# wsakobe/CylinderTag

Measured on AMD Instinct MI355X. Metric: frames/sec detect() 1920x1080, higher is better.
Workload: dtype u8; 1 GPU; synthetic 1920x1080 random-stripe frames, 4096 per step over 1 GPU(s), 4 planted CTag_2f12c markers each, detect(img,5,true,5), inputs resident in HBM; frames_per_gpu=4096, chunk=4096, parallelism=frames sharded, dp1, gather=none (1 GPU)

## Files before the change

### __graft_entry__.py

```python
import os
import subprocess
import sys

ROOT = os.path.dirname(os.path.abspath(__file__))
if ROOT not in sys.path:
    sys.path.insert(0, ROOT)


def build():
    subprocess.check_call(["make", "-s", "-j4", "-C", os.path.join(ROOT, "cylindertag_amd")])
    for name, extra in (("hedge", "-DCTAG_WELSCH_MINERR_IN_LOOP -DCTAG_RESIZE_SIMD_LANES=16"), ("plainsync", "-DCTAG_REFINE_PLAIN_SYNC=1")):
        out = os.path.join("_var", name)
        subprocess.check_call(["make", "-s", "-j4", "-C", os.path.join(ROOT, "cylindertag_amd"), "OUT=" + out, "EXTRA=" + extra, os.path.join(out, "libctag_hip.so")])
    subprocess.check_call(["make", "-s", "-C", os.path.join(ROOT, "testkit")])
    subprocess.check_call(["make", "-s", "-C", os.path.join(ROOT, "oracle")])
    if os.path.isdir("/root/reference"):
        subprocess.call(["make", "-s", "-C", os.path.join(ROOT, "oracle"), "ref"])
    import cylindertag_amd
    from cylindertag_amd import capi
    L = capi.load_library()
    missing = [s for s in capi.EXPORTS if not hasattr(L, s)]
    if missing:
        raise RuntimeError("libctag_hip.so lacks symbols: %s" % missing)
    import testkit
    T = testkit.load_library()
    missing = [s for s in testkit.EXPORTS if not hasattr(T, s)]
# ... 48 lines not shown
```

### cylindertag_amd/csrc/ctag_internal.h

```cpp
#pragma once
#include <hip/hip_runtime.h>
#include <stddef.h>
#include <stdint.h>

#include <vector>

#include "../../include/ctag_types.h"

struct ctag_handle;
struct ctag_camera;
struct ctag_pose_rec;
struct ctag_rig_pose_rec;
struct ctag_mv_pose_rec;
struct ctag_camera_set;

namespace ctag {
template <class T>
struct DevBuf {
    T* p = nullptr;
    size_t cap = 0;
    DevBuf() = default;
    DevBuf(const DevBuf&) = delete;
    DevBuf& operator=(const DevBuf&) = delete;
    ~DevBuf() { release(); }
// ... 292 lines not shown
ChunkPlan plan_chunk(const PlanIn& in);

hipError_t launch_zero_counters(const ChunkPlan& pl, const Workspace& ws, hipStream_t s);
hipError_t launch_decimate(const ChunkPlan& pl, const uint8_t* frames, ptrdiff_t frame_stride, ptrdiff_t row_stride, const Workspace& ws, hipStream_t s);
hipError_t launch_threshold_ccl(const ChunkPlan& pl, const Workspace& ws, hipStream_t s);
hipError_t launch_seam_merge(const ChunkPlan& pl, const Workspace& ws, hipStream_t s);
hipError_t launch_resolve(const ChunkPlan& pl, const Workspace& ws, hipStream_t s);
hipError_t launch_candidates(const ChunkPlan& pl, const Workspace& ws, hipStream_t s);
hipError_t launch_quads(const ChunkPlan& pl, const Workspace& ws, hipStream_t s, hipEvent_t* ev5 = nullptr);
hipError_t launch_line_fits(const ChunkPlan& pl, const Workspace& ws, hipStream_t s, unsigned long long* stamps = nullptr, hipEvent_t ev_sorted = nullptr);
int welsch_limits(int32_t* out, int capacity);
hipError_t launch_features(const ChunkPlan& pl, const Workspace& ws, const DetectParams& p, hipStream_t s);
hipError_t launch_edge_refine(const ChunkPlan& pl, const uint8_t* frames, ptrdiff_t frame_stride, ptrdiff_t row_stride, const Workspace& ws, const DetectParams& p, hipStream_t s);
hipError_t launch_edge_refine_sums(const ChunkPlan& pl, const Workspace& ws, hipStream_t s);
hipError_t launch_markers(const ChunkPlan& pl, const Workspace& ws, const DetectParams& p, ctag_frame_result* out, const PendingCtx& pend, hipStream_t s);
hipError_t launch_counters(int nframes, const Workspace& ws, const ctag_frame_result* results, long long* out10, hipStream_t s);
size_t threshold_ccl_lds_bytes(int tw);
bool build_threshold_table(float dark_cap, uint8_t* table , int* dim, int* tcap);
void build_pick_table(uint8_t* table, uint16_t* table16);


enum SiblingState { kPoseState, kDrawState, kRigState, kGatherState, kMvState, kCovState, kFitState, kRigFitState, kCamFitState, kIntrFitState, kRobustState, kTrackState, kHandEyeState, kNumSiblingStates };
void** handle_state_slot(struct ::ctag_handle* h, SiblingState which, void (*free_fn)(void*));
int model_to_device(struct ::ctag_model* m, int device);
int rigs_to_device(struct ::ctag_rigs* r, int device);
bool camera_ok(const struct ::ctag_camera* c);
bool handle_timing(const struct ::ctag_handle* h);
int handle_finish_pending(struct ::ctag_handle* h);
bool handle_pending_state(struct ::ctag_handle* h, const int32_t** count_dev, uint64_t* gen);
void handle_pending_clean(struct ::ctag_handle* h, uint64_t gen);
// ... 46 lines not shown
```

### cylindertag_amd/csrc/k_feature.hip

```cpp
#include "ctag_internal.h"
#include "ctag_math.h"
#include "ctag_refine.h"
#include "ctag_wave.h"

namespace ctag {

constexpr double kPi = 3.1415926535897932384626433832795;

struct P2 {
    float x, y;
};
__device__ __forceinline__ float dist2p(P2 a, P2 b) { return ctm::sqrt32((a.x - b.x) * (a.x - b.x) + (a.y - b.y) * (a.y - b.y)); }
__device__ __forceinline__ double angdeg(float dy, float dx) { return ctm::atan2_32(dy, dx) * 180 / kPi; }

struct QuadDerived {
    float cx, cy, d[4], a1, a2;
    float e[4];
};
static_assert(sizeof(QuadDerived) == 48, "workspace carve in ctag_api.hip");
struct FeatPtrs {
    const int32_t* ncand;
    const QuadOut* quads;
    QuadDerived* derived;
    int32_t* quad_index;
// ... 377 lines not shown
        f2[k] = F;
    }
    clk.mark(5);
}

struct RefinePtrs {
    const uint8_t* frames;
    ptrdiff_t frame_stride, row_stride;
    const int32_t* nfeat;
    const int32_t* status;
    const FeatureDev* feat1;
    FeatureDev* feat2;
    double* n0;
    int32_t* frame_long;
    int ch;
};
static RefinePtrs refine_ptrs(const uint8_t* frames, ptrdiff_t frame_stride, ptrdiff_t row_stride, const Workspace& ws, const DetectParams& p) {
    RefinePtrs P{};
    P.frames = frames, P.frame_stride = frame_stride, P.row_stride = row_stride, P.ch = p.channels == 3 ? 3 : 1;
    P.nfeat = ws.nfeat, P.status = ws.status, P.feat1 = ws.feat1, P.feat2 = ws.feat2, P.n0 = ws.refine_n0, P.frame_long = ws.frame_long;
    return P;
}
constexpr int kRefineSamples = 128;
constexpr int kRefineThreads = 2 * kRefineSamples;
#ifndef CTAG_REFINE_STAGE_DEEP
#define CTAG_REFINE_STAGE_DEEP 12
#endif
#ifndef CTAG_REFINE_REGION
#define CTAG_REFINE_REGION 21504
#endif
constexpr int kRefineRegion = CTAG_REFINE_REGION;
#ifndef CTAG_REFINE_REGION_LARGE
#define CTAG_REFINE_REGION_LARGE 49152
#endif
constexpr int kRefineRegionLarge = CTAG_REFINE_REGION_LARGE;

#ifndef CTAG_REFINE_SEARCH_WAVES
#define CTAG_REFINE_SEARCH_WAVES 4
#endif
__device__ __forceinline__ void refine_line(const double* A, double* L) {
    const double Mx = A[0], My = A[1], Mxx = A[2], Mxy = A[3], Myy = A[4], N = A[5];
    const ctm::Recip64 RN = ctm::recip64(N);
    const double Ex = ctm::div64(Mx, RN), Ey = ctm::div64(My, RN);
    const double Cxx = ctm::div64(Mxx, RN) - Ex * Ex;
    const double Cxy = ctm::div64(Mxy, RN) - Ex * Ey;
    const double Cyy = ctm::div64(Myy, RN) - Ey * Ey;
    const double normal_theta = .5 * ctm::atan2_32((float)(-2 * Cxy), (float)(Cyy - Cxx));
    L[0] = Ex;
    L[1] = Ey;
    float sn, cs;
    ctm::sincos32((float)normal_theta, &sn, &cs);
// ... 15 lines not shown
        O->c[2 * idx] = (float)(Ln[0] + L0 * A00);
        O->c[2 * idx + 1] = (float)(Ln[1] + L0 * A10);
    } else {
        O->c[2 * idx] = F->c[2 * idx];
        O->c[2 * idx + 1] = F->c[2 * idx + 1];
    }
}

#if defined(CTAG_REFINE_PLAIN_SYNC) && CTAG_REFINE_PLAIN_SYNC
__device__ __forceinline__ void refine_sync() { __syncthreads(); }
__device__ __forceinline__ void sums_sync() { __syncthreads(); }
#else
__device__ __forceinline__ void refine_sync() { lds_barrier(); }
__device__ __forceinline__ void sums_sync() { lds_wait(), __builtin_amdgcn_s_waitcnt(0xc07f); }
#endif
template <int MODE, int REGION = kRefineRegion>
__device__ __forceinline__ bool refine_quad(const RefinePtrs& P, int rows, int cols, int subpix, int frame, int qidx, int only_long, double alpha128 = 0.0) {
    constexpr int kPitch = kRefineSamples + 1;
    constexpr int kRows = 16;
#ifndef CTAG_ONES_SHIFT
#define CTAG_ONES_SHIFT 16
#endif
    __shared__ __attribute__((aligned(16))) double s_vall[MODE == 1 ? kPitch : (kRows + 1) * kPitch + CTAG_ONES_SHIFT];
    double (*s_v)[kPitch] = reinterpret_cast<double (*)[kPitch]>(s_vall);
    double* const s_ones = MODE == 1 ? s_vall : s_vall + kRows * kPitch + CTAG_ONES_SHIFT;
    double (*s_bx)[kPitch] = s_v, (*s_by)[kPitch] = s_v + (MODE == 1 ? 0 : 4);
    __shared__ double s_nrm[4][2];
    __shared__ uint64_t s_step[4][2];
    __shared__ double s_acc[48];
    __shared__ __attribute__((aligned(16))) uint8_t s_reg[REGION];
    const int fi = qidx >> 1, quad = qidx & 1;
    const int tid = threadIdx.x;
    const FeatureDev* F = P.feat1 + (size_t)frame * CTAG_MAX_FEATURES + fi;
    const uint8_t* __restrict__ img = P.frames + (ptrdiff_t)frame * P.frame_stride;
    const uint32_t rs = (uint32_t)P.row_stride;
    const int off = quad * 4;
    __shared__ float s_cx[4], s_cy[4];
    __shared__ int s_ns[4];
    __shared__ int s_box[4];
    if (tid < 4) {
        s_cx[tid] = F->c[2 * (off + tid)];
        s_cy[tid] = F->c[2 * (off + tid) + 1];
    }
    double* const accp = s_acc;
    if (MODE != 1 && tid < 48) accp[tid] = 0.0;
    if constexpr (MODE != 1) {
        for (int k = tid; k < kPitch; k += (int)blockDim.x) s_ones[k] = 1.0;
    }
    refine_sync();
    if (tid < 4) {
        const int a = tid, b = (tid + 1) & 3;
        const double nx = s_cy[b] - s_cy[a];
        const double ny = -s_cx[b] + s_cx[a];
        const double mag = ctm::sqrt64(nx * nx + ny * ny);
        const double ns_d = mag / 8 > 128.0 ? mag / 8 : 128.0;
        s_ns[tid] = (int)ns_d;
        s_nrm[tid][0] = nx / mag;
        s_nrm[tid][1] = ny / mag;
        s_step[tid][0] = ctr::fast_step(nx / mag);
        s_step[tid][1] = ctr::fast_step(ny / mag);
    }
    if (tid == 64) {
        const float m = (float)(subpix + 3);
        const float fx0 = fminf(fminf(s_cx[0], s_cx[1]), fminf(s_cx[2], s_cx[3])) - m, fx1 = fmaxf(fmaxf(s_cx[0], s_cx[1]), fmaxf(s_cx[2], s_cx[3])) + m;
        const float fy0 = fminf(fminf(s_cy[0], s_cy[1]), fminf(s_cy[2], s_cy[3])) - m, fy1 = fmaxf(fmaxf(s_cy[0], s_cy[1]), fmaxf(s_cy[2], s_cy[3])) + m;
        int staged = 0, bx0 = 0, by0 = 0, pitch = 4;
        if (fx0 > -1e6f && fx1 < 1e6f && fy0 > -1e6f && fy1 < 1e6f) {
            bx0 = max((int)floorf(fx0), 0) & ~3;
            by0 = max((int)floorf(fy0), 0);
            const int bx1 = min((int)floorf(fx1) + 1, cols - 1), by1 = min((int)floorf(fy1) + 1, rows - 1);
            if (bx1 >= bx0 && by1 >= by0) {
                pitch = (bx1 - bx0 + 4) & ~3;
                if (((pitch >> 2) & 1) == 0) pitch += 4;
                staged = ((long long)pitch * (by1 - by0 + 1) <= REGION && (pitch >> 2) <= kRefineThreads) ? by1 - by0 + 1 : 0;
            }
        }
        s_box[0] = bx0;
        s_box[1] = by0;
        s_box[2] = pitch;
        s_box[3] = staged;
    }
    refine_sync();
    const int max_ns = max(max(s_ns[0], s_ns[1]), max(s_ns[2], s_ns[3]));
    {
        const bool long_quad = max_ns > kRefineSamples;
        if (MODE == 1 && long_quad && tid == 0) P.frame_long[frame] = 1;
        if (MODE != 0 && long_quad) return false;
        if (MODE == 0 && only_long && !long_quad) return false;
    }
    const int box_x0 = s_box[0], box_y0 = s_box[1], box_pitch = s_box[2], box_rows = s_box[3];
    const bool staged = box_rows > 0;
    if (staged) {
        const int wpr = box_pitch >> 2;
        const int rpp = kRefineThreads / wpr;
        const bool aligned = ((rs & 3u) == 0u) && ((reinterpret_cast<uintptr_t>(img) & 3u) == 0u);
        const int r0 = tid / wpr, c4 = (tid - r0 * wpr) * 4;
        const int gx = box_x0 + c4;
        if (rpp > 0 && r0 < rpp) {
            auto stage_rows = [&](auto load, auto conv) {
                int r = r0;
                if constexpr (MODE == 1) {
                    constexpr int kDeep = CTAG_REFINE_STAGE_DEEP;
                    for (; r + (kDeep - 1) * rpp < box_rows; r += kDeep * rpp) {
                        decltype(load(0)) v[kDeep];
#pragma unroll
                        for (int u = 0; u < kDeep; u++) v[u] = load(r + u * rpp);
#pragma unroll
                        for (int u = 0; u < kDeep; u++) *reinterpret_cast<uint32_t*>(s_reg + (r + u * rpp) * box_pitch + c4) = conv(v[u]);
                    }
                }
                for (; r + 3 * rpp < box_rows; r += 4 * rpp) {
                    const auto v0 = load(r), v1 = load(r + rpp), v2 = load(r + 2 * rpp), v3 = load(r + 3 * rpp);
                    *reinterpret_cast<uint32_t*>(s_reg + r * box_pitch + c4) = conv(v0);
                    *reinterpret_cast<uint32_t*>(s_reg + (r + rpp) * box_pitch + c4) = conv(v1);
                    *reinterpret_cast<uint32_t*>(s_reg + (r + 2 * rpp) * box_pitch + c4) = conv(v2);
                    *reinterpret_cast<uint32_t*>(s_reg + (r + 3 * rpp) * box_pitch + c4) = conv(v3);
                }
                for (; r < box_rows; r += rpp) *reinterpret_cast<uint32_t*>(s_reg + r * box_pitch + c4) = conv(load(r));
            };
            auto same = [](uint32_t v) -> uint32_t { return v; };
            if (P.ch == 3) {
                struct W3 {
                    uint32_t a, b, c;
                };
                if (aligned && box_x0 + box_pitch <= cols) {
                    stage_rows(
                        [&](int r) -> W3 {
                            const uint32_t* src = reinterpret_cast<const uint32_t*>(img + (size_t)__umul24((unsigned)(box_y0 + r), rs) + 3 * gx);
                            return W3{src[0], src[1], src[2]};
                        },
                        [](const W3& w) -> uint32_t { return gray4_of(w.a, w.b, w.c); });
                } else {
                    stage_rows(
                        [&](int r) -> uint32_t {
                            const uint8_t* src = img + (size_t)__umul24((unsigned)(box_y0 + r), rs) + 3 * gx;
                            uint32_t v = 0;
// ... 22 lines not shown
    const int half = tid >> 7, st = tid & (kRefineSamples - 1);
    double* const n0_quad = P.n0 + ((size_t)frame * (CTAG_MAX_FEATURES * 2) + qidx) * (4 * kRefineSamples);
    for (int sbase = 0; sbase < max_ns; sbase += kRefineSamples) {
        const int s = sbase + st;
#pragma nounroll
        for (int epair = 0; epair < 2; epair++) {
            const int edge = 2 * epair + half;
            const int a = edge, b = (edge + 1) & 3;
            const float ax = s_cx[a], ay = s_cy[a], bx = s_cx[b], by = s_cy[b];
            const int nsamples = s_ns[edge];
            const double nx = s_nrm[edge][0], ny = s_nrm[edge][1];
            const bool axis = nx == 0.0 || ny == 0.0;
            const uint64_t step_xy[2] = {s_step[edge][0], s_step[edge][1]};
            bool ok = false;
            double bestx = 0, besty = 0, alpha = 0;
            if (s < nsamples) {
                alpha = MODE == 1 ? alpha128 : (15.0 + s) / (nsamples + 30);
                const double x0 = alpha * ax + (1 - alpha) * bx;
                const double y0 = alpha * ay + (1 - alpha) * by;
                double Mn = 0, Mcount = 0;
                const bool bgr = P.ch == 3;
                auto px = [&](int x, int y) -> unsigned {
                    if (bgr) {
                        const uint8_t* q = img + __umul24((unsigned)y, rs) + 3u * (unsigned)x;
                        return gray_of(q[0], q[1], q[2]);
                    }
                    return img[__umul24((unsigned)y, rs) + (unsigned)x];
                };
                bool done = false;
                if (subpix <= ctr::kFastMaxSubpix && ctr::interior(x0, y0, nx, ny, subpix, rows, cols)) {
                    if (staged) {
                        auto px_lds = [&](int x, int y) -> unsigned { return s_reg[__umul24((unsigned)y, (unsigned)box_pitch) + (unsigned)x]; };
                        if (!axis)
                            done = subpix == 5 ? ctr::search_fast<5>(x0, y0, nx, ny, 5, px_lds, Mn, Mcount, box_x0, box_y0, step_xy)
                                               : ctr::search_fast<0>(x0, y0, nx, ny, subpix, px_lds, Mn, Mcount, box_x0, box_y0, step_xy);
                        if (!done) {
                            ctr::search_mid<0>(x0, y0, nx, ny, subpix, px_lds, Mn, Mcount, box_x0, box_y0);
                            done = true;
                        }
                    } else {
                        done = ctr::search_fast(x0, y0, nx, ny, subpix, px, Mn, Mcount);
                    }
                }
                if (!done) ctr::search_exact(x0, y0, nx, ny, subpix, rows, cols, px, Mn, Mcount);
                if (Mcount != 0) {
                    const double n0 = Mn / Mcount;
                    bestx = x0 + n0 * nx;
                    besty = y0 + n0 * ny;
                    ok = true;
                    if constexpr (MODE == 1) n0_quad[edge * kRefineSamples + st] = n0;
                }
            }
            if constexpr (MODE == 1) {
                if (!ok) n0_quad[edge * kRefineSamples + st] = ctm::bits_to_f64(0x7ff8000000000000ULL);
            } else {
                s_bx[edge][st] = bestx;
                s_by[edge][st] = besty;
                s_v[8 + edge][st] = ok ? 1 - alpha : 0.0;
                s_v[12 + edge][st] = ok ? alpha : 0.0;
            }
        }
        if constexpr (MODE == 1) return false;
        refine_sync();
        if (tid < 48) {
            const int edge = tid / 12, r = tid - edge * 12;
// ... 12 lines not shown
            }
            for (; k < cntS; k++) acc += (pa[k] * pb[k]) * pw[k];
            accp[tid] = acc;
        }
        refine_sync();
    }
    if (tid < 8) {
        const int edge = tid >> 1, pass = tid & 1;
        refine_line(s_acc + edge * 12 + pass * 6, s_acc + edge * 12 + pass * 6);
    }
    refine_sync();
    if (tid < 4) refine_corner(s_acc, tid, off, F, P.feat2 + (size_t)frame * CTAG_MAX_FEATURES + fi);
    return true;
}

template <int MODE, int REGION = kRefineRegion>
__global__ __launch_bounds__(kRefineThreads) __attribute__((amdgpu_waves_per_eu(MODE == 1 ? (REGION > 36864 ? 3 : CTAG_REFINE_SEARCH_WAVES) : 1, MODE == 1 ? CTAG_REFINE_SEARCH_WAVES : 8)))
void k_edge_refine(RefinePtrs P, int rows, int cols, int subpix, int nframes, int per_frame) {
    int frame = blockIdx.y, bx = blockIdx.x, gx = gridDim.x;
    if (per_frame > 0) {
        const int b = blockIdx.x;
        frame = ((b >> 3) / per_frame) * 8 + (b & 7);
        bx = (b >> 3) % per_frame;
        gx = per_frame;
    }
    if (frame >= nframes) return;
    if (P.status[frame] != CTAG_OK) return;
    const int nq = 2 * min(P.nfeat[frame], CTAG_MAX_FEATURES);
    const double alpha128 = (15.0 + (double)((int)threadIdx.x & (kRefineSamples - 1))) / (kRefineSamples + 30);
    for (int q = bx; q < nq; q += gx) {
        refine_quad<MODE, REGION>(P, rows, cols, subpix, frame, q, 0, alpha128);
        if (q + gx < nq) refine_sync();
    }
}
#ifndef CTAG_REFINE_SUMS2_WAVES
#define CTAG_REFINE_SUMS2_WAVES 4
#endif
constexpr int kSumSeg = 16, kSumSegs = kRefineSamples / kSumSeg;
constexpr int kSumPitch = kSumSeg + 2;
constexpr int kSumRows = 24;
struct SumsWeights {
    double w[kRefineSamples][2];
    constexpr SumsWeights() : w{} {
        for (int s = 0; s < kRefineSamples; s++) {
            const double alpha = (15.0 + s) / (kRefineSamples + 30);
            w[s][0] = 1 - alpha;
// ... 838 lines not shown
            }
            out_markers++;
            out_features += rn;
        }
        clk.mark(24);
    }
    if (tid == 0) {
        out->status = CTAG_OK;
        out->n_markers = out_markers;
        out->n_features = out_features;
        out->flags = oflags;
    }
}

static Stamps feat_stamps;

hipError_t launch_features(const ChunkPlan& pl, const Workspace& ws, const DetectParams& p, hipStream_t s) {
    const FeatPtrs P = feat_ptrs(ws, pl.feat_stamps ? feat_stamps.zeroed(s) : nullptr);
    if (pl.latency) hipLaunchKernelGGL(k_features<512>, dim3(pl.nframes), dim3(512), 0, s, P, pl.nframes, p.feature_size);
    else hipLaunchKernelGGL(k_features<128>, dim3(pl.nframes), dim3(128), 0, s, P, pl.nframes, p.feature_size);
    return hipGetLastError();
}
static void launch_refine_sums(const ChunkPlan& pl, const RefinePtrs& P, hipStream_t s) {
    const int f8 = ((pl.nframes + 7) / 8) * 8;
    hipLaunchKernelGGL(k_edge_refine_sums, dim3(f8 * pl.refine_sums_gx), dim3(64), 0, s, P, pl.nframes, pl.refine_sums_gx);
}
hipError_t launch_edge_refine_sums(const ChunkPlan& pl, const Workspace& ws, hipStream_t s) {
    launch_refine_sums(pl, refine_ptrs(nullptr, 0, 0, ws, DetectParams{}), s);
    return hipGetLastError();
}
hipError_t launch_edge_refine(const ChunkPlan& pl, const uint8_t* frames, ptrdiff_t frame_stride, ptrdiff_t row_stride, const Workspace& ws, const DetectParams& p, hipStream_t s) {
    const int nframes = pl.nframes, refine_gx = pl.refine_gx, f8 = ((nframes + 7) / 8) * 8;
    const RefinePtrs P = refine_ptrs(frames, frame_stride, row_stride, ws, p);
    if (pl.refine == RefineForm::None) return hipSuccess;
    if (pl.refine == RefineForm::One) {
        hipLaunchKernelGGL(k_edge_refine<0>, dim3(CTAG_MAX_FEATURES * 2, nframes), dim3(kRefineThreads), 0, s, P, ws.g.rows, ws.g.cols, p.subpix_dist, nframes, 0);
        return hipGetLastError();
    }
    if (pl.refine == RefineForm::SplitLarge) hipLaunchKernelGGL((k_edge_refine<1, kRefineRegionLarge>), dim3(f8 * refine_gx), dim3(kRefineThreads), 0, s, P, ws.g.rows, ws.g.cols, p.subpix_dist, nframes, refine_gx);
    else if (pl.refine == RefineForm::SplitLooping) hipLaunchKernelGGL(k_edge_refine<1>, dim3(f8 * refine_gx), dim3(kRefineThreads), 0, s, P, ws.g.rows, ws.g.cols, p.subpix_dist, nframes, refine_gx);
    else hipLaunchKernelGGL(k_edge_refine<1>, dim3(refine_gx, nframes), dim3(kRefineThreads), 0, s, P, ws.g.rows, ws.g.cols, p.subpix_dist, nframes, 0);
    launch_refine_sums(pl, P, s);
    hipLaunchKernelGGL(k_edge_refine_tail, dim3(13, nframes), dim3(64), 0, s, P, nframes, 13);
    hipLaunchKernelGGL(k_edge_refine_long, dim3(4, nframes), dim3(kRefineThreads), 0, s, P, ws.g.rows, ws.g.cols, p.subpix_dist, nframes);
    return hipGetLastError();
}
hipError_t launch_markers(const ChunkPlan& pl, const Workspace& ws, const DetectParams& p, ctag_frame_result* out, const PendingCtx& pend, hipStream_t s) {
    const MarkerPtrs P = marker_ptrs(ws, p, out, pend, pl.feat_stamps ? feat_stamps.d : nullptr);
    if (pl.latency) hipLaunchKernelGGL(k_markers<8>, dim3(pl.nframes), dim3(512), 0, s, P, pl.nframes, p.feature_size, p.dict_rows, p.dict_cols);
    else hipLaunchKernelGGL(k_markers<1>, dim3(pl.nframes), dim3(64), 0, s, P, pl.nframes, p.feature_size, p.dict_rows, p.dict_cols);
    if (pl.feat_stamps) {
        unsigned long long h[25];
        feat_stamps.read(s, h, 25);
        fprintf(stderr, "[k_features ticks] compact %llu derive %llu pairs %llu greedy %llu organise %llu obtain %llu\n", h[0], h[1], h[2], h[3], h[4], h[5]);
        fprintf(stderr, "[k_markers ticks] load %llu pairs %llu union %llu sort %llu ids %llu carry+pre %llu | code %llu coverage %llu pick+store %llu\n", h[16], h[17], h[18],
                h[19], h[20], h[21], h[22], h[23], h[24]);
    }
    return hipGetLastError();
}

}
```

### include/ctag_testkit.h

```cpp
#ifndef CTAG_TESTKIT_H
#define CTAG_TESTKIT_H
#include <stddef.h>
#include <stdint.h>

#include "ctag.h"
#include "ctag_pose.h"

#ifdef __cplusplus
extern "C" {
#endif

#define CTAG_DBG_HALF 1
#define CTAG_DBG_LABELS 2
#define CTAG_DBG_CANDIDATES 3
#define CTAG_DBG_CAND_QUADS 4
#define CTAG_DBG_FEATURES0 5
#define CTAG_DBG_FEATURES1 6
#define CTAG_DBG_FEATURES2 7
#define CTAG_DBG_PREMARKERS 8
#define CTAG_DBG_GRAY 9
#define CTAG_DBG_MASK 11
#define CTAG_DBG_LINES 10
#define CTAG_DBG_LINE_POINTS 12
#define CTAG_DBG_LINE_FITS 13
// ... 72 lines not shown
                            ctag_synth3d_truth* truth);
int ctag_synth3d_model(const int32_t* state, int dict_rows, int dict_cols, float* corners);

int ctag_testkit_dense_edge_probe(ctag_handle* h, const uint8_t* gray, int rows, int cols, ptrdiff_t row_stride, const double* segments,
                                  int n_seg, const double* K, const double* dist, const double* rvec, const double* tvec,
                                  int samples_per_edge, double search_px, double min_contrast, double* out, int32_t* keep);

int ctag_testkit_welsch_fit(ctag_handle* h, int n_frames, const int32_t* edges_per_frame, const int32_t* points_per_edge, const int32_t* xy,
                            int latency, int welsch_gx, int welsch_gs, int tail_at_pool_end, float* lines);

int ctag_testkit_welsch_limits(int32_t* out, int capacity);

int ctag_testkit_refine_sums(ctag_handle* h, int n_frames, const int32_t* nfeat, const int32_t* status, const float* corners, const double* n0,
                             double* sums);

int ctag_testkit_model_fit_system(ctag_handle* h, const ctag_frame_result* results, int n_frames, const ctag_pose_rec* poses, int n_poses,
                                  const ctag_model* model, const ctag_camera* camera, int model_index, double lambda, int min_obs, int pass_records,
                                  double* S, double* g, double* delta, int32_t* held, int32_t* bad_pivot);
int ctag_testkit_model_fit_limits(int32_t* out, int capacity);

int ctag_testkit_rig_fit_system(ctag_handle* h, const ctag_frame_result* results, int n_frames, const ctag_rig_pose_rec* rig_poses,
                                const ctag_model* model, const ctag_rigs* rigs, const ctag_camera* camera, int rig, double lambda, int pass_records,
                                double* S, double* g, double* delta, int32_t* n_unknowns, int32_t* bad_pivot);
int ctag_testkit_rig_fit_limits(int32_t* out, int capacity);

int ctag_testkit_camera_fit_system(ctag_handle* h, const ctag_frame_result* results, int n_frames, const ctag_mv_pose_rec* mv_poses,
                                   const ctag_model* model, const ctag_rigs* rigs, const ctag_camera_set* cams, int anchor, double lambda,
                                   int pass_records, double* S, double* g, double* delta, int32_t* n_unknowns, int32_t* bad_pivot);
int ctag_testkit_camera_fit_limits(int32_t* out, int capacity);

// ... 16 lines not shown
```

### testkit/__init__.py

```python
import ctypes as C
import os
import subprocess

import numpy as np

import cylindertag_amd as ca
from cylindertag_amd import capi
from cylindertag_amd.capi import CtagError, Model

_HERE = os.path.dirname(os.path.abspath(__file__))
_LIB = os.environ.get("CTAG_TESTKIT_LIB") or os.path.join(_HERE, "_build", "libctag_testkit.so")

TRUTH3D_DT = np.dtype([("n_markers", "<i4"), ("dict_row", "<i4", (8,)), ("_pad", "<i4", (1,)), ("R", "<f8", (8, 9)), ("t", "<f8", (8, 3)),
                       ("radius", "<f8", (8,))])
TRUTH_DT = np.dtype([("n_markers", "<i4"), ("dict_row", "<i4", (8,)), ("strip_len", "<f4", (8,)),
                     ("corners", "<f4", (8, 8))])
DBG_HALF, DBG_LABELS, DBG_CANDIDATES, DBG_CAND_QUADS, DBG_FEATURES0, DBG_FEATURES1, DBG_FEATURES2, DBG_PREMARKERS, DBG_GRAY, DBG_LINES, DBG_MASK, DBG_LINE_POINTS, DBG_LINE_FITS, DBG_PACKS, DBG_PACKS1 = range(1, 16)
SYNTH_SEED = 0x4354616753594E00

EXPORTS = ["ctag_debug_fetch", "ctag_math_probe", "ctag_testkit_wave_probe", "ctag_testkit_exp32_k0_sweep", "ctag_testkit_unpack_gathered", "ctag_testkit_stall_stream", "ctag_synth_frames_device", "ctag_synth_frame_host",
           "ctag_synth_layout_truth", "ctag_synth3d_frames_device", "ctag_synth3d_frame_host", "ctag_synth3d_model",
           "ctag_testkit_dense_edge_probe", "ctag_testkit_plan", "ctag_testkit_welsch_fit", "ctag_testkit_welsch_limits", "ctag_testkit_refine_sums",
           "ctag_testkit_model_fit_system", "ctag_testkit_model_fit_limits", "ctag_testkit_rig_fit_system", "ctag_testkit_rig_fit_limits",
           "ctag_testkit_camera_fit_system", "ctag_testkit_camera_fit_limits",
           "ctag_testkit_intrinsics_fit_system", "ctag_testkit_intrinsics_fit_poses", "ctag_testkit_intrinsics_fit_limits"]
PLAN_FIELDS = ("fused", "bgr_direct", "zero_first", "dec_zero_kernel", "dec_zero_list", "dec", "dec_xblocks", "dec_yblocks", "dec_band_rows", "dec_bands",
               "ccl", "latency", "small_cfg", "refprm", "mask_scan", "prescan", "all_wave", "fork", "pack_max", "big_points", "pack_gx", "scan_gx",
               "mscan_gx", "big_cols", "big_max_gx", "welsch_gs", "welsch_gx", "refine", "refine_gx", "refine_sums_gx")
DEC_FORMS = ("mask", "mask_bands", "general", "wide", "banded135", "banded", "unaligned")
CCL_FORMS = ("mask", "tw5", "any")
WELSCH_LIMITS = ("kWShort", "kWCap", "kWRes", "kWPts", "kWPtsU", "kPickN", "kPickN2", "kWE", "kWT", "kLatLines", "kLatPoints", "kLatChunk", "kLdsLines",
                 "kLatencyFrames", "kLatRankBlocks", "kLineSortBuckets")
REFINE_FORMS = ("none", "one", "split_large", "split_looping", "split")
MATH_EXP32_NONPOS, MATH_EXP32_NONPOS_K0, MATH_LOG64 = 15, 17, 18
WAVE_OPS = ("FROM_PREV", "FROM_NEXT", "SHR1_I32", "SHR2_I32", "SHR4_I32", "SHR1_F32", "SHR1_F64", "XOR1_I32", "XOR2_I32", "HALF_MIRROR_I32", "ROW_MIRROR_I32",
            "XOR1_I64", "XOR2_I64", "HALF_MIRROR_I64", "ROW_MIRROR_I64", "INCL_SCAN", "SG_SUM8_I32", "SG_SUM64_I32", "SG_SUM8_I64", "SG_SUM64_I64",
            "SG_BEST8_NEAREST", "SG_BEST8_FARTHEST", "SG_BEST64_NEAREST", "SG_BEST64_FARTHEST", "SUM_F64", "MAX_F64", "ALL", "PK_MIN_U16", "PK_MAX_U16")
for _i, _n in enumerate(WAVE_OPS):
    globals()["WAVE_" + _n] = _i
WAVE_SENTINEL_F64, WAVE_SENTINEL_I64 = -12345.6789, -0x5a5a5a5a5a5a5a5a


def lib_path():
    return _LIB


def build(verbose=False):
# ... 39 lines not shown
    L.ctag_synth3d_frame_host.restype = C.c_int
    L.ctag_synth3d_frame_host.argtypes = [i32p, C.c_int, C.c_int, vp, C.c_int, C.c_int, C.c_int, C.c_ssize_t, C.c_uint64, C.c_int, C.c_double,
                                          C.c_double, C.c_double, C.c_double, vp]
    L.ctag_synth3d_model.restype = C.c_int
    L.ctag_synth3d_model.argtypes = [i32p, C.c_int, C.c_int, vp]
    L.ctag_testkit_plan.restype = C.c_int
    L.ctag_testkit_plan.argtypes = [C.c_int, C.c_int, C.c_int, C.c_int, C.c_int, C.c_int, vp, C.c_ssize_t, C.c_ssize_t, C.c_int, C.c_int, C.c_int,
                                    C.c_int, i32p, C.c_int]
    L.ctag_testkit_dense_edge_probe.restype = C.c_int
    L.ctag_testkit_dense_edge_probe.argtypes = [vp, vp, C.c_int, C.c_int, C.c_ssize_t, vp, C.c_int, vp, vp, vp, vp, C.c_int,
                                                C.c_double, C.c_double, vp, vp]
    L.ctag_testkit_welsch_fit.restype = C.c_int
    L.ctag_testkit_welsch_fit.argtypes = [vp, C.c_int, vp, vp, vp, C.c_int, C.c_int, C.c_int, C.c_int, vp]
    L.ctag_testkit_refine_sums.restype = C.c_int
    L.ctag_testkit_refine_sums.argtypes = [vp, C.c_int, vp, vp, vp, vp, vp]
    L.ctag_testkit_welsch_limits.restype = C.c_int
    L.ctag_testkit_welsch_limits.argtypes = [i32p, C.c_int]
    L.ctag_testkit_model_fit_system.restype = C.c_int
    L.ctag_testkit_model_fit_system.argtypes = [vp, vp, C.c_int, vp, C.c_int, vp, C.POINTER(capi.CameraC), C.c_int, C.c_double, C.c_int, C.c_int, vp, vp, vp,
                                                vp, i32p]
    L.ctag_testkit_model_fit_limits.restype = C.c_int
    L.ctag_testkit_model_fit_limits.argtypes = [i32p, C.c_int]
    L.ctag_testkit_rig_fit_system.restype = C.c_int
    L.ctag_testkit_rig_fit_system.argtypes = [vp, vp, C.c_int, vp, vp, vp, C.POINTER(capi.CameraC), C.c_int, C.c_double, C.c_int, vp, vp, vp, i32p, i32p]
    L.ctag_testkit_rig_fit_limits.restype = C.c_int
    L.ctag_testkit_rig_fit_limits.argtypes = [i32p, C.c_int]
    L.ctag_testkit_camera_fit_system.restype = C.c_int
    L.ctag_testkit_camera_fit_system.argtypes = [vp, vp, C.c_int, vp, vp, vp, vp, C.c_int, C.c_double, C.c_int, vp, vp, vp, i32p, i32p]
    L.ctag_testkit_camera_fit_limits.restype = C.c_int
    L.ctag_testkit_camera_fit_limits.argtypes = [i32p, C.c_int]
# ... 108 lines not shown
                            bgr_direct, expand_exact, out.ctypes.data_as(C.POINTER(C.c_int32)), len(out))
    if n != len(PLAN_FIELDS):
        raise RuntimeError("ctag_testkit_plan writes %d fields, PLAN_FIELDS names %d" % (n, len(PLAN_FIELDS)))
    plan = dict(zip(PLAN_FIELDS, (int(v) for v in out)))
    plan["dec"], plan["ccl"], plan["refine"] = DEC_FORMS[plan["dec"]], CCL_FORMS[plan["ccl"]], REFINE_FORMS[plan["refine"]]
    return plan


def welsch_limits():
    L = load_library()
    out = np.zeros(len(WELSCH_LIMITS), np.int32)
    n = L.ctag_testkit_welsch_limits(out.ctypes.data_as(C.POINTER(C.c_int32)), len(out))
    if n != len(WELSCH_LIMITS):
        raise RuntimeError("ctag_testkit_welsch_limits writes %d values, WELSCH_LIMITS names %d" % (n, len(WELSCH_LIMITS)))
    return dict(zip(WELSCH_LIMITS, (int(v) for v in out)))


class Detector(ca.Detector):

    def __init__(self, state, feature_size, device=0, **kw):
        super().__init__(state, feature_size, device=device, **kw)
        self.T = load_library()

    def synth_frames_device(self, frames_ptr, first, n, rows, cols, row_stride, frame_stride, seed=SYNTH_SEED, markers=4):
        st = self.T.ctag_synth_frames_device(self.h, frames_ptr, first, n, rows, cols, row_stride, frame_stride, seed, markers)
        if st != 0:
            raise CtagError(st, "ctag_synth_frames_device")

    def synth3d_frames_device(self, frames_ptr, first, n, rows, cols, row_stride, frame_stride, K, seed=SYNTH_SEED, markers=4):
        K = np.asarray(K, np.float64)
# ... 176 lines not shown
```

### testkit/ctag_testkit.hip

```cpp
#include <hip/hip_runtime.h>

#include <algorithm>
#include <cstring>
#include <vector>

#include "../include/ctag_testkit.h"
#include "../cylindertag_amd/csrc/ctag_internal.h"
#include "../cylindertag_amd/csrc/ctag_math.h"
#include "../cylindertag_amd/csrc/ctag_wave.h"
#include "ctag_synth.h"

using namespace ctag;

#define TK_TRY(expr)                              \
    do {                                          \
        if ((expr) != hipSuccess) return CTAG_ERR_HIP; \
    } while (0)

namespace {

__global__ void k_math_probe(int op, int n, const double* a, const double* b, double* out) {
    const int i = blockIdx.x * blockDim.x + threadIdx.x;
    if (i >= n) return;
    const double x = a[i], y = b[i];
// ... 820 lines not shown
    if (launch_edge_refine_sums(pl, W, s) != hipSuccess) {
        (void)hipGetLastError();
        return CTAG_ERR_HIP;
    }
    TK_TRY(hipStreamSynchronize(s));
    f0 = 0;
    for (int f = 0; f < n_frames; f++) {
        const size_t nq = (size_t)nfeat[f] * 2;
        if (nq == 0) continue;
        TK_TRY(hipMemcpy2D(sums + f0 * 49, 49 * 8, W.refine_n0 + (size_t)f * (CTAG_MAX_FEATURES * 2) * kQuad, kQuad * 8, 49 * 8, nq, hipMemcpyDeviceToHost));
        f0 += nq;
    }
    return CTAG_OK;
}

int ctag_testkit_model_fit_system(ctag_handle* h, const ctag_frame_result* results, int n_frames, const ctag_pose_rec* poses, int n_poses,
                                  const ctag_model* model, const ctag_camera* camera, int model_index, double lambda, int min_obs, int pass_records,
                                  double* S, double* g, double* delta, int32_t* held, int32_t* bad_pivot) {
    return mfit_probe_system(h, results, n_frames, poses, n_poses, model, camera, model_index, lambda, min_obs, pass_records, S, g, delta, held, bad_pivot);
}

int ctag_testkit_model_fit_limits(int32_t* out, int capacity) {
    const int32_t v[2] = {mfit_record_grid(), mfit_pass_records()};
    if (out) std::memcpy(out, v, sizeof(int32_t) * (size_t)std::min(std::max(capacity, 0), 2));
    return 2;
}

int ctag_testkit_rig_fit_system(ctag_handle* h, const ctag_frame_result* results, int n_frames, const ctag_rig_pose_rec* rig_poses,
                                const ctag_model* model, const ctag_rigs* rigs, const ctag_camera* camera, int rig, double lambda, int pass_records,
                                double* S, double* g, double* delta, int32_t* n_unknowns, int32_t* bad_pivot) {
// ... 58 lines not shown
```

Before: 291,400 frames/s.

## Stage sheared LDS windows for slanted quads and enlarge search region

For the search-mode refine kernel, quads whose bounding box is too large to stage now try a sheared window along the dominant edge direction. Each row is offset by an integer shear, so slanted edges fit in LDS and avoid the global-memory/exact search path. The default search-region LDS budget is also raised, and optional path counters are added for profiling. The cost is more LDS per block, which may reduce occupancy, plus extra setup arithmetic per quad.

```diff
diff --git a/__graft_entry__.py b/__graft_entry__.py
--- a/__graft_entry__.py
+++ b/__graft_entry__.py
@@ -9,7 +9,8 @@
 
 def build():
     subprocess.check_call(["make", "-s", "-j4", "-C", os.path.join(ROOT, "cylindertag_amd")])
-    for name, extra in (("hedge", "-DCTAG_WELSCH_MINERR_IN_LOOP -DCTAG_RESIZE_SIMD_LANES=16"), ("plainsync", "-DCTAG_REFINE_PLAIN_SYNC=1")):
+    for name, extra in (("hedge", "-DCTAG_WELSCH_MINERR_IN_LOOP -DCTAG_RESIZE_SIMD_LANES=16"), ("plainsync", "-DCTAG_REFINE_PLAIN_SYNC=1"),
+                        ("region12k", "-DCTAG_REFINE_SEARCH_REGION=12288")):
         out = os.path.join("_var", name)
         subprocess.check_call(["make", "-s", "-j4", "-C", os.path.join(ROOT, "cylindertag_amd"), "OUT=" + out, "EXTRA=" + extra, os.path.join(out, "libctag_hip.so")])
     subprocess.check_call(["make", "-s", "-C", os.path.join(ROOT, "testkit")])
diff --git a/cylindertag_amd/csrc/ctag_internal.h b/cylindertag_amd/csrc/ctag_internal.h
--- a/cylindertag_amd/csrc/ctag_internal.h
+++ b/cylindertag_amd/csrc/ctag_internal.h
@@ -330,6 +330,7 @@
 hipError_t launch_edge_refine(const ChunkPlan& pl, const uint8_t* frames, ptrdiff_t frame_stride, ptrdiff_t row_stride, const Workspace& ws, const DetectParams& p, hipStream_t s);
 hipError_t launch_edge_refine_sums(const ChunkPlan& pl, const Workspace& ws, hipStream_t s);
 hipError_t launch_markers(const ChunkPlan& pl, const Workspace& ws, const DetectParams& p, ctag_frame_result* out, const PendingCtx& pend, hipStream_t s);
+int refine_path_counts(unsigned long long* out, int capacity, int reset);
 hipError_t launch_counters(int nframes, const Workspace& ws, const ctag_frame_result* results, long long* out10, hipStream_t s);
 size_t threshold_ccl_lds_bytes(int tw);
 bool build_threshold_table(float dark_cap, uint8_t* table , int* dim, int* tcap);
diff --git a/cylindertag_amd/csrc/k_feature.hip b/cylindertag_amd/csrc/k_feature.hip
--- a/cylindertag_amd/csrc/k_feature.hip
+++ b/cylindertag_amd/csrc/k_feature.hip
@@ -415,6 +415,7 @@
     double* n0;
     int32_t* frame_long;
     int ch;
+    unsigned long long* stamps;
 };
 static RefinePtrs refine_ptrs(const uint8_t* frames, ptrdiff_t frame_stride, ptrdiff_t row_stride, const Workspace& ws, const DetectParams& p) {
     RefinePtrs P{};
@@ -431,11 +432,19 @@
 #define CTAG_REFINE_REGION 21504
 #endif
 constexpr int kRefineRegion = CTAG_REFINE_REGION;
+constexpr int kRefineSearchFour = 39936;
+#ifndef CTAG_REFINE_SEARCH_REGION
+#define CTAG_REFINE_SEARCH_REGION kRefineSearchFour
+#endif
+constexpr int kRefineSearchRegion = CTAG_REFINE_SEARCH_REGION;
 #ifndef CTAG_REFINE_REGION_LARGE
 #define CTAG_REFINE_REGION_LARGE 49152
 #endif
 constexpr int kRefineRegionLarge = CTAG_REFINE_REGION_LARGE;
 
+#ifndef CTAG_REFINE_SHEAR
+#define CTAG_REFINE_SHEAR 1
+#endif
 #ifndef CTAG_REFINE_SEARCH_WAVES
 #define CTAG_REFINE_SEARCH_WAVES 4
 #endif
@@ -481,7 +490,9 @@
 __device__ __forceinline__ void refine_sync() { lds_barrier(); }
 __device__ __forceinline__ void sums_sync() { lds_wait(), __builtin_amdgcn_s_waitcnt(0xc07f); }
 #endif
-template <int MODE, int REGION = kRefineRegion>
+enum RefineCount { kCountPlain, kCountSheared, kCountUnstaged, kCountFast, kCountMid, kCountExact, kCountDeclined, kRefineCounts };
+constexpr int kRefineCountSlot = 6;
+template <int MODE, int REGION = kRefineRegion, bool COUNT = false>
 __device__ __forceinline__ bool refine_quad(const RefinePtrs& P, int rows, int cols, int subpix, int frame, int qidx, int only_long, double alpha128 = 0.0) {
     constexpr int kPitch = kRefineSamples + 1;
     constexpr int kRows = 16;
@@ -504,7 +515,7 @@
     const int off = quad * 4;
     __shared__ float s_cx[4], s_cy[4];
     __shared__ int s_ns[4];
-    __shared__ int s_box[4];
+    __shared__ int s_box[6];
     if (tid < 4) {
         s_cx[tid] = F->c[2 * (off + tid)];
         s_cy[tid] = F->c[2 * (off + tid) + 1];
@@ -531,7 +542,7 @@
         const float m = (float)(subpix + 3);
         const float fx0 = fminf(fminf(s_cx[0], s_cx[1]), fminf(s_cx[2], s_cx[3])) - m, fx1 = fmaxf(fmaxf(s_cx[0], s_cx[1]), fmaxf(s_cx[2], s_cx[3])) + m;
         const float fy0 = fminf(fminf(s_cy[0], s_cy[1]), fminf(s_cy[2], s_cy[3])) - m, fy1 = fmaxf(fmaxf(s_cy[0], s_cy[1]), fmaxf(s_cy[2], s_cy[3])) + m;
-        int staged = 0, bx0 = 0, by0 = 0, pitch = 4;
+        int staged = 0, bx0 = 0, by0 = 0, pitch = 4, mult = 4, shear = 0;
         if (fx0 > -1e6f && fx1 < 1e6f && fy0 > -1e6f && fy1 < 1e6f) {
             bx0 = max((int)floorf(fx0), 0) & ~3;
             by0 = max((int)floorf(fy0), 0);
@@ -540,12 +551,36 @@
                 pitch = (bx1 - bx0 + 4) & ~3;
                 if (((pitch >> 2) & 1) == 0) pitch += 4;
                 staged = ((long long)pitch * (by1 - by0 + 1) <= REGION && (pitch >> 2) <= kRefineThreads) ? by1 - by0 + 1 : 0;
+                mult = pitch;
+                if (MODE == 1 && CTAG_REFINE_SHEAR && !staged) {
+                    float len = -1.f, dx = 0.f, dy = 0.f;
+                    for (int i = 0; i < 4; i++) {
+                        const float ex = s_cx[(i + 1) & 3] - s_cx[i], ey = s_cy[(i + 1) & 3] - s_cy[i];
+                        const float l = ex * ex + ey * ey;
+                        if (l > len) len = l, dx = ex, dy = ey;
+                    }
+                    const float q = dy != 0.f ? dx / dy : 1e9f;
+                    const int k = fabsf(q) < 4.5f ? (int)rintf(q) : 0;
+                    if (k != 0) {
+                        const float fk = (float)k, mk = m * (1.f + fabsf(fk));
+                        float umin = 3e38f, umax = -3e38f;
+                        for (int i = 0; i < 4; i++) {
+                            const float u = s_cx[i] - fk * (s_cy[i] - (float)by0);
+                            umin = fminf(umin, u), umax = fmaxf(umax, u);
+                        }
+                        const int u0 = (int)floorf(umin - mk) - 1, u1 = (int)floorf(umax + mk) + 2, nr = by1 - by0 + 1;
+                        const int ps = (u1 - u0 + 4) & ~3;
+                        if ((long long)ps * nr <= REGION && (ps >> 2) <= kRefineThreads && ps - k >= 1) staged = nr, bx0 = u0, pitch = ps, mult = ps - k, shear = k;
+                    }
+                }
             }
         }
         s_box[0] = bx0;
         s_box[1] = by0;
-        s_box[2] = pitch;
+        s_box[2] = mult;
         s_box[3] = staged;
+        s_box[4] = pitch;
+        s_box[5] = shear;
     }
     refine_sync();
     const int max_ns = max(max(s_ns[0], s_ns[1]), max(s_ns[2], s_ns[3]));
@@ -555,8 +590,12 @@
         if (MODE != 0 && long_quad) return false;
         if (MODE == 0 && only_long && !long_quad) return false;
     }
-    const int box_x0 = s_box[0], box_y0 = s_box[1], box_pitch = s_box[2], box_rows = s_box[3];
+    const int box_x0 = s_box[0], box_y0 = s_box[1], box_rows = s_box[3], box_pitch = s_box[4];
+    const int box_mult = MODE == 1 ? s_box[2] : box_pitch, box_shear = MODE == 1 ? s_box[5] : 0;
     const bool staged = box_rows > 0;
+    if constexpr (COUNT) {
+        if (tid == 0) atomicAdd(&P.stamps[kRefineCountSlot + (staged ? (box_shear != 0 ? kCountSheared : kCountPlain) : kCountUnstaged)], 1ull);
+    }
     if (staged) {
         const int wpr = box_pitch >> 2;
         const int rpp = kRefineThreads / wpr;
@@ -586,7 +625,34 @@
                 for (; r < box_rows; r += rpp) *reinterpret_cast<uint32_t*>(s_reg + r * box_pitch + c4) = conv(load(r));
             };
             auto same = [](uint32_t v) -> uint32_t { return v; };
-            if (P.ch == 3) {
+            if (box_shear != 0) {
+                const int xlast = box_x0 + box_shear * (box_rows - 1);
+                const bool inside = P.ch == 1 && min(box_x0, xlast) >= 0 && max(box_x0, xlast) + box_pitch <= cols;
+                if (inside) {
+                    stage_rows(
+                        [&](int r) -> uint32_t {
+                            uint32_t v;
+                            __builtin_memcpy(&v, img + (size_t)__umul24((unsigned)(box_y0 + r), rs) + (unsigned)(gx + box_shear * r), 4);
+                            return v;
+                        },
+                        same);
+                } else {
+                    const bool bgr3 = P.ch == 3;
+                    stage_rows(
+                        [&](int r) -> uint32_t {
+                            const uint8_t* row = img + (size_t)__umul24((unsigned)(box_y0 + r), rs);
+                            const int x = gx + box_shear * r;
+                            uint32_t v = 0;
+                            for (int k = 0; k < 4; k++)
+                                if ((unsigned)(x + k) < (unsigned)cols) {
+                                    const uint8_t* q = row + (bgr3 ? 3 * (x + k) : x + k);
+                                    v |= (bgr3 ? gray_of(q[0], q[1], q[2]) : (uint32_t)q[0]) << (8 * k);
+                                }
+                            return v;
+                        },
+                        same);
+                }
+            } else if (P.ch == 3) {
                 struct W3 {
                     uint32_t a, b, c;
                 };
@@ -639,6 +705,7 @@
             const uint64_t step_xy[2] = {s_step[edge][0], s_step[edge][1]};
             bool ok = false;
             double bestx = 0, besty = 0, alpha = 0;
+            int path = -1;
             if (s < nsamples) {
                 alpha = MODE == 1 ? alpha128 : (15.0 + s) / (nsamples + 30);
                 const double x0 = alpha * ax + (1 - alpha) * bx;
@@ -655,25 +722,36 @@
                 bool done = false;
                 if (subpix <= ctr::kFastMaxSubpix && ctr::interior(x0, y0, nx, ny, subpix, rows, cols)) {
                     if (staged) {
-                        auto px_lds = [&](int x, int y) -> unsigned { return s_reg[__umul24((unsigned)y, (unsigned)box_pitch) + (unsigned)x]; };
+                        auto px_lds = [&](int x, int y) -> unsigned { return s_reg[__umul24((unsigned)y, (unsigned)box_mult) + (unsigned)x]; };
                         if (!axis)
                             done = subpix == 5 ? ctr::search_fast<5>(x0, y0, nx, ny, 5, px_lds, Mn, Mcount, box_x0, box_y0, step_xy)
                                                : ctr::search_fast<0>(x0, y0, nx, ny, subpix, px_lds, Mn, Mcount, box_x0, box_y0, step_xy);
+                        if constexpr (COUNT) path = done ? kCountFast : (axis ? kCountMid : kCountDeclined);
                         if (!done) {
                             ctr::search_mid<0>(x0, y0, nx, ny, subpix, px_lds, Mn, Mcount, box_x0, box_y0);
                             done = true;
                         }
                     } else {
                         done = ctr::search_fast(x0, y0, nx, ny, subpix, px, Mn, Mcount);
+                        if constexpr (COUNT) path = kCountFast;
                     }
                 }
-                if (!done) ctr::search_exact(x0, y0, nx, ny, subpix, rows, cols, px, Mn, Mcount);
+                if (!done) {
+                    ctr::search_exact(x0, y0, nx, ny, subpix, rows, cols, px, Mn, Mcount);
+                    if constexpr (COUNT) path = kCountExact;
+                }
                 if (Mcount != 0) {
                     const double n0 = Mn / Mcount;
                     bestx = x0 + n0 * nx;
                     besty = y0 + n0 * ny;
                     ok = true;
                     if constexpr (MODE == 1) n0_quad[edge * kRefineSamples + st] = n0;
+                }
+            }
+            if constexpr (COUNT) {
+                for (int k = kCountFast; k < kRefineCounts; k++) {
+                    const unsigned long long took = __ballot(path == k);
+                    if (took != 0 && (tid & 63) == 0) atomicAdd(&P.stamps[kRefineCountSlot + k], (unsigned long long)__popcll(took));
                 }
             }
             if constexpr (MODE == 1) {
@@ -716,8 +794,8 @@
     return true;
 }
 
-template <int MODE, int REGION = kRefineRegion>
-__global__ __launch_bounds__(kRefineThreads) __attribute__((amdgpu_waves_per_eu(MODE == 1 ? (REGION > 36864 ? 3 : CTAG_REFINE_SEARCH_WAVES) : 1, MODE == 1 ? CTAG_REFINE_SEARCH_WAVES : 8)))
+template <int MODE, int REGION = kRefineRegion, bool COUNT = false>
+__global__ __launch_bounds__(kRefineThreads) __attribute__((amdgpu_waves_per_eu(MODE == 1 ? (REGION > kRefineSearchFour ? 3 : CTAG_REFINE_SEARCH_WAVES) : 1, MODE == 1 ? CTAG_REFINE_SEARCH_WAVES : 8)))
 void k_edge_refine(RefinePtrs P, int rows, int cols, int subpix, int nframes, int per_frame) {
     int frame = blockIdx.y, bx = blockIdx.x, gx = gridDim.x;
     if (per_frame > 0) {
@@ -731,7 +809,7 @@
     const int nq = 2 * min(P.nfeat[frame], CTAG_MAX_FEATURES);
     const double alpha128 = (15.0 + (double)((int)threadIdx.x & (kRefineSamples - 1))) / (kRefineSamples + 30);
     for (int q = bx; q < nq; q += gx) {
-        refine_quad<MODE, REGION>(P, rows, cols, subpix, frame, q, 0, alpha128);
+        refine_quad<MODE, REGION, COUNT>(P, rows, cols, subpix, frame, q, 0, alpha128);
         if (q + gx < nq) refine_sync();
     }
 }
@@ -1600,6 +1678,19 @@
 }
 
 static Stamps feat_stamps;
+static unsigned long long refine_counts_total[kRefineCounts];
+
+int refine_path_counts(unsigned long long* out, int capacity, int reset) {
+    for (int k = 0; k < kRefineCounts && k < capacity; k++) out[k] = refine_counts_total[k];
+    for (int k = 0; reset && k < kRefineCounts; k++) refine_counts_total[k] = 0;
+    return kRefineCounts;
+}
+template <int REGION>
+static void launch_refine_search(const ChunkPlan& pl, RefinePtrs P, dim3 grid, const Workspace& ws, const DetectParams& p, int per_frame, hipStream_t s) {
+    P.stamps = pl.feat_stamps ? feat_stamps.d : nullptr;
+    if (P.stamps) hipLaunchKernelGGL((k_edge_refine<1, REGION, true>), grid, dim3(kRefineThreads), 0, s, P, ws.g.rows, ws.g.cols, p.subpix_dist, pl.nframes, per_frame);
+    else hipLaunchKernelGGL((k_edge_refine<1, REGION>), grid, dim3(kRefineThreads), 0, s, P, ws.g.rows, ws.g.cols, p.subpix_dist, pl.nframes, per_frame);
+}
 
 hipError_t launch_features(const ChunkPlan& pl, const Workspace& ws, const DetectParams& p, hipStream_t s) {
     const FeatPtrs P = feat_ptrs(ws, pl.feat_stamps ? feat_stamps.zeroed(s) : nullptr);
@@ -1623,9 +1714,9 @@
         hipLaunchKernelGGL(k_edge_refine<0>, dim3(CTAG_MAX_FEATURES * 2, nframes), dim3(kRefineThreads), 0, s, P, ws.g.rows, ws.g.cols, p.subpix_dist, nframes, 0);
         return hipGetLastError();
     }
-    if (pl.refine == RefineForm::SplitLarge) hipLaunchKernelGGL((k_edge_refine<1, kRefineRegionLarge>), dim3(f8 * refine_gx), dim3(kRefineThreads), 0, s, P, ws.g.rows, ws.g.cols, p.subpix_dist, nframes, refine_gx);
-    else if (pl.refine == RefineForm::SplitLooping) hipLaunchKernelGGL(k_edge_refine<1>, dim3(f8 * refine_gx), dim3(kRefineThreads), 0, s, P, ws.g.rows, ws.g.cols, p.subpix_dist, nframes, refine_gx);
-    else hipLaunchKernelGGL(k_edge_refine<1>, dim3(refine_gx, nframes), dim3(kRefineThreads), 0, s, P, ws.g.rows, ws.g.cols, p.subpix_dist, nframes, 0);
+    if (pl.refine == RefineForm::SplitLarge) launch_refine_search<kRefineRegionLarge>(pl, P, dim3(f8 * refine_gx), ws, p, refine_gx, s);
+    else if (pl.refine == RefineForm::SplitLooping) launch_refine_search<kRefineSearchRegion>(pl, P, dim3(f8 * refine_gx), ws, p, refine_gx, s);
+    else launch_refine_search<kRefineSearchRegion>(pl, P, dim3(refine_gx, nframes), ws, p, 0, s);
     launch_refine_sums(pl, P, s);
     hipLaunchKernelGGL(k_edge_refine_tail, dim3(13, nframes), dim3(64), 0, s, P, nframes, 13);
     hipLaunchKernelGGL(k_edge_refine_long, dim3(4, nframes), dim3(kRefineThreads), 0, s, P, ws.g.rows, ws.g.cols, p.subpix_dist, nframes);
@@ -1638,6 +1729,10 @@
     if (pl.feat_stamps) {
         unsigned long long h[25];
         feat_stamps.read(s, h, 25);
+        const unsigned long long* c = h + kRefineCountSlot;
+        for (int k = 0; k < kRefineCounts; k++) refine_counts_total[k] += c[k];
+        fprintf(stderr, "k_edge_refine<1> paths: quads: plain %llu sheared %llu unstaged %llu | samples: fast %llu mid %llu exact %llu declined->mid %llu\n", c[kCountPlain],
+                c[kCountSheared], c[kCountUnstaged], c[kCountFast], c[kCountMid], c[kCountExact], c[kCountDeclined]);
         fprintf(stderr, "[k_features ticks] compact %llu derive %llu pairs %llu greedy %llu organise %llu obtain %llu\n", h[0], h[1], h[2], h[3], h[4], h[5]);
         fprintf(stderr, "[k_markers ticks] load %llu pairs %llu union %llu sort %llu ids %llu carry+pre %llu | code %llu coverage %llu pick+store %llu\n", h[16], h[17], h[18],
                 h[19], h[20], h[21], h[22], h[23], h[24]);
diff --git a/include/ctag_testkit.h b/include/ctag_testkit.h
--- a/include/ctag_testkit.h
+++ b/include/ctag_testkit.h
@@ -110,6 +110,8 @@
 int ctag_testkit_refine_sums(ctag_handle* h, int n_frames, const int32_t* nfeat, const int32_t* status, const float* corners, const double* n0,
                              double* sums);
 
+int ctag_testkit_refine_paths(uint64_t* out, int capacity, int reset);
+
 int ctag_testkit_model_fit_system(ctag_handle* h, const ctag_frame_result* results, int n_frames, const ctag_pose_rec* poses, int n_poses,
                                   const ctag_model* model, const ctag_camera* camera, int model_index, double lambda, int min_obs, int pass_records,
                                   double* S, double* g, double* delta, int32_t* held, int32_t* bad_pivot);
diff --git a/testkit/__init__.py b/testkit/__init__.py
--- a/testkit/__init__.py
+++ b/testkit/__init__.py
@@ -21,6 +21,7 @@
 EXPORTS = ["ctag_debug_fetch", "ctag_math_probe", "ctag_testkit_wave_probe", "ctag_testkit_exp32_k0_sweep", "ctag_testkit_unpack_gathered", "ctag_testkit_stall_stream", "ctag_synth_frames_device", "ctag_synth_frame_host",
            "ctag_synth_layout_truth", "ctag_synth3d_frames_device", "ctag_synth3d_frame_host", "ctag_synth3d_model",
            "ctag_testkit_dense_edge_probe", "ctag_testkit_plan", "ctag_testkit_welsch_fit", "ctag_testkit_welsch_limits", "ctag_testkit_refine_sums",
+           "ctag_testkit_refine_paths",
            "ctag_testkit_model_fit_system", "ctag_testkit_model_fit_limits", "ctag_testkit_rig_fit_system", "ctag_testkit_rig_fit_limits",
            "ctag_testkit_camera_fit_system", "ctag_testkit_camera_fit_limits",
            "ctag_testkit_intrinsics_fit_system", "ctag_testkit_intrinsics_fit_poses", "ctag_testkit_intrinsics_fit_limits"]
@@ -31,6 +32,7 @@
 CCL_FORMS = ("mask", "tw5", "any")
 WELSCH_LIMITS = ("kWShort", "kWCap", "kWRes", "kWPts", "kWPtsU", "kPickN", "kPickN2", "kWE", "kWT", "kLatLines", "kLatPoints", "kLatChunk", "kLdsLines",
                  "kLatencyFrames", "kLatRankBlocks", "kLineSortBuckets")
+REFINE_PATHS = ("quads_plain", "quads_sheared", "quads_unstaged", "fast", "mid", "exact", "declined_mid")
 REFINE_FORMS = ("none", "one", "split_large", "split_looping", "split")
 MATH_EXP32_NONPOS, MATH_EXP32_NONPOS_K0, MATH_LOG64 = 15, 17, 18
 WAVE_OPS = ("FROM_PREV", "FROM_NEXT", "SHR1_I32", "SHR2_I32", "SHR4_I32", "SHR1_F32", "SHR1_F64", "XOR1_I32", "XOR2_I32", "HALF_MIRROR_I32", "ROW_MIRROR_I32",
@@ -100,6 +102,8 @@
     L.ctag_testkit_welsch_fit.argtypes = [vp, C.c_int, vp, vp, vp, C.c_int, C.c_int, C.c_int, C.c_int, vp]
     L.ctag_testkit_refine_sums.restype = C.c_int
     L.ctag_testkit_refine_sums.argtypes = [vp, C.c_int, vp, vp, vp, vp, vp]
+    L.ctag_testkit_refine_paths.restype = C.c_int
+    L.ctag_testkit_refine_paths.argtypes = [C.POINTER(C.c_uint64), C.c_int, C.c_int]
     L.ctag_testkit_welsch_limits.restype = C.c_int
     L.ctag_testkit_welsch_limits.argtypes = [i32p, C.c_int]
     L.ctag_testkit_model_fit_system.restype = C.c_int
@@ -238,6 +242,14 @@
     if n != len(WELSCH_LIMITS):
         raise RuntimeError("ctag_testkit_welsch_limits writes %d values, WELSCH_LIMITS names %d" % (n, len(WELSCH_LIMITS)))
     return dict(zip(WELSCH_LIMITS, (int(v) for v in out)))
+
+
+def refine_paths(reset=True):
+    out = np.zeros(len(REFINE_PATHS), np.uint64)
+    n = load_library().ctag_testkit_refine_paths(out.ctypes.data_as(C.POINTER(C.c_uint64)), len(out), int(bool(reset)))
+    if n != len(REFINE_PATHS):
+        raise RuntimeError("ctag_testkit_refine_paths writes %d values, REFINE_PATHS names %d" % (n, len(REFINE_PATHS)))
+    return dict(zip(REFINE_PATHS, (int(v) for v in out)))
 
 
 class Detector(ca.Detector):
diff --git a/testkit/ctag_testkit.hip b/testkit/ctag_testkit.hip
--- a/testkit/ctag_testkit.hip
+++ b/testkit/ctag_testkit.hip
@@ -858,6 +858,13 @@
     return CTAG_OK;
 }
 
+int ctag_testkit_refine_paths(uint64_t* out, int capacity, int reset) {
+    unsigned long long v[16] = {};
+    const int n = refine_path_counts(v, 16, reset);
+    for (int k = 0; out && k < n && k < capacity; k++) out[k] = v[k];
+    return n;
+}
+
 int ctag_testkit_model_fit_system(ctag_handle* h, const ctag_frame_result* results, int n_frames, const ctag_pose_rec* poses, int n_poses,
                                   const ctag_model* model, const ctag_camera* camera, int model_index, double lambda, int min_obs, int pass_records,
                                   double* S, double* g, double* delta, int32_t* held, int32_t* bad_pivot) {
```

After: 292,200 frames/s, median of 6. About the same (+0.3%).
